# davidfischinger/haf_grasping

Hardware: NVIDIA B200
Metric: grasp_windows_scored_per_sec_all_rolls (higher is better)
Workload: dtype f32 (contraction: fp16 operands, 1 tensor-core product per k-slice, f32 accumulate; f64 guard band)

## Files before the change

haf_grasping_b200/csrc/hafgpu.cu:

```cuda
#include <cuda_runtime.h>

#include <algorithm>
#include <cmath>
#include <cstdarg>
#include <cstdio>
#include <condition_variable>
#include <cstring>
#include <mutex>
#include <unordered_map>
#include <string>
#include <thread>
#include <vector>

#include "../../include/hafgpu.h"
#include "haf_host.hpp"
#include "host/pcd_io.hpp"
#include "kernels.cuh"
#include "pcd_ingest.cuh"
#include "svm_tc.cuh"

using namespace hafk;

static thread_local std::string g_create_error;

// ... 591 lines not shown
        {
            const int forced = (cfg->reserved[0] >> 4) & 3;
            double rel[4] = {0, 0, 0, 0};
            if (!forced || cfg->guard_rel <= 0) calibrate_tensor_passes(model, Dsv, rel);
            int passes = 3;
            if (forced) passes = forced;
            else if (rel[1] <= 5.5e-7) passes = 1;
            else if (rel[2] <= 5.5e-7) passes = 2;
            ctx->tc_passes = passes;
            ctx->tc_operand_err = passes < 3 ? rel[passes] : 0.0;
            if (cfg->guard_rel <= 0) ctx->guard_rel = std::max(4e-6f, (float)(15.0 * (ctx->tc_operand_err + 2.5e-7)));
        }
        if (!make_tensor_map(&ctx->tmSh2, ctx->d_SVh.p, KB, SpadT) || !make_tensor_map(&ctx->tmSl2, ctx->d_SVl.p, KB, SpadT)) {
            haf_destroy(ctx);
            return create_fail(HAF_ERR_CUDA, "cuTensorMapEncodeTiled failed for the support-vector operands");
        }
        std::vector<DimFeat> joined((size_t)32 * D);
        for (int cls = 0; cls < 32; cls++)
        for (int d = 0; d < D; d++) {
            DimFeat j;
            memset(&j, 0, sizeof j);
            const DimDev& dd = dims[d];
            if (dd.feat >= 0) {
                const FeatDev& ff = fd[dd.feat];
                for (int r = 0; r < 3; r++) {
                    if (ff.flags & (1 << r)) {
                        for (int q = 0; q < 4; q++) {
                            const int x = ff.off[4 * r + q] / ld, y = ff.off[4 * r + q] % ld;
                            j.off[4 * r + q] = (x * (ld + cls) + y) * 4;
                        }
                        j.w[r] = ff.w[r];
                    } else {
                        for (int q = 0; q < 4; q++) j.off[4 * r + q] = 0;
                        j.w[r] = 0.0f;
                    }
                }
                j.flags = ff.flags & 0x104;
            } else {
                j.flags = 0x200;
            }
            if (dd.drop) j.flags |= 0x400;
            j.fmin = (float)dd.fmin; j.slope = (float)dd.slope; j.cval = (float)dd.cval;
            joined[(size_t)cls * D + d] = j;
        }
        Round4Tab r4;
        make_round4_table(r4);
        if (ctx->d_round4.ensure(1) != 0) { haf_destroy(ctx); return create_fail(HAF_ERR_NOMEM, "out of device memory uploading the rounding table"); }
        CREATE_TRY(cudaMemcpy(ctx->d_round4.p, &r4, sizeof(Round4Tab), cudaMemcpyHostToDevice));
        if (ctx->d_dimfeat.ensure(joined.size()) != 0) { haf_destroy(ctx); return create_fail(HAF_ERR_NOMEM, "out of device memory uploading the joined feature table"); }
        CREATE_TRY(cudaMemcpy(ctx->d_dimfeat.p, joined.data(), joined.size() * sizeof(DimFeat), cudaMemcpyHostToDevice));
        CREATE_TRY(cudaFuncSetAttribute(haftc::svm_rbf_tc2_kernel, cudaFuncAttributeMaxDynamicSharedMemorySize, haftc::SMEM2_BYTES + haftc::TAB_SMEM_MAX * 4));
        CREATE_TRY(cudaFuncSetAttribute(haftc::svm_rbf_tc3_kernel<2>, cudaFuncAttributeMaxDynamicSharedMemorySize, haftc::TC3_SMEM_LIMIT));
        CREATE_TRY(cudaFuncSetAttribute(haftc::svm_rbf_tc3_kernel<4>, cudaFuncAttributeMaxDynamicSharedMemorySize, haftc::TC3_SMEM_LIMIT));
        CREATE_TRY(cudaFuncSetAttribute(features_tc_kernel, cudaFuncAttributeMaxDynamicSharedMemorySize, (int)ft_smem_layout(G, 2)));
        CREATE_TRY(cudaFuncSetAttribute(features_tc_kernel, cudaFuncAttributePreferredSharedMemoryCarveout, 90));
    }
    for (int i = 0; i < 10; i++) CREATE_TRY(cudaEventCreate(&ctx->ev[i]));
    ctx->ev_ok = true;
#undef CREATE_TRY
    *out = ctx;
    return HAF_OK;
}

extern "C" int haf_create(haf_ctx** out, const haf_config* cfg) {
    if (!out || !cfg) return create_fail(HAF_ERR_ARG, "haf_create: null argument");
    if (cfg->n_devices <= 1) {
        haf_config one = *cfg;
        if (cfg->n_devices == 1 && cfg->devices) one.device = cfg->devices[0];
        one.n_devices = 0; one.devices = nullptr;
        return create_impl(out, &one, false, 0);
    }
    *out = nullptr;
    if (cfg->n_devices > 64) return create_fail(HAF_ERR_ARG, "haf_create: n_devices out of range");
    std::vector<haf_ctx*> members;
    for (int k = 0; k < cfg->n_devices; k++) {
        haf_config one = *cfg;
        one.device = cfg->devices ? cfg->devices[k] : k;
        one.n_devices = 0; one.devices = nullptr;
        for (size_t j = 0; j < members.size(); j++)
            if (members[j]->device == one.device) {
                for (size_t i = 0; i < members.size(); i++) haf_destroy(members[i]);
                return create_fail(HAF_ERR_ARG, "haf_create: devices[] names the same GPU twice");
            }
        haf_ctx* c = nullptr;
        const int rc = create_impl(&c, &one, false, 0);
        if (rc != HAF_OK) {
            for (size_t i = 0; i < members.size(); i++) haf_destroy(members[i]);
            return rc;
        }
        members.push_back(c);
    }
    members[0]->group = members;
    *out = members[0];
    return HAF_OK;
}

static int svm_stage(haf_ctx* ctx, unsigned* cnt, size_t Wcap, size_t ldx, int G, int ubase, cudaStream_t st, cudaEvent_t ev_guard);
extern "C" int haf_svm_create(haf_svm** out, const char* model_path, int device, int svm_mode, int min_dims, float guard_rel) {
    haf_config cfg;
    memset(&cfg, 0, sizeof cfg);
    cfg.model_path = model_path;
    cfg.device = device;
    cfg.svm_mode = svm_mode;
    cfg.guard_rel = guard_rel;
    const int rc = create_impl(out, &cfg, true, min_dims);
    if (rc == HAF_OK) (*out)->svm_only = true;
    return rc;
}
// ... 263 lines not shown

extern "C" int haf_build_transform(const haf_request* req, int roll, int roll_step_deg, float M[16]) {
    if (!req || !M) return HAF_ERR_ARG;
    hafhost::build_transform(*req, roll, roll_step_deg > 0 ? roll_step_deg : 15, M);
    return HAF_OK;
}
extern "C" int haf_build_transform_wcs(const haf_request* req, int roll, int roll_step_deg, float M[16]) {
    if (!req || !M) return HAF_ERR_ARG;
    hafhost::build_transform_wcs(*req, roll, roll_step_deg > 0 ? roll_step_deg : 15, M);
    return HAF_OK;
}
extern "C" int haf_pack_best_records(const haf_best* best, int n, int32_t* records) {
    if (!best || !records || n < 0) return HAF_ERR_ARG;
    for (int i = 0; i < n; i++) {
        int32_t* r = records + (size_t)i * 8;
        r[0] = best[i].topval; r[1] = best[i].row; r[2] = best[i].col; r[3] = best[i].roll; r[4] = best[i].tilt;
        r[5] = best[i].approach_idx; r[6] = best[i].n_windows_scored; r[7] = best[i].rolls_done;
    }
    return HAF_OK;
}
extern "C" uint64_t haf_best_key(int topval, uint32_t unit_order) {
    return ((uint64_t)(uint32_t)(topval + (1 << 30)) << 32) | (uint64_t)(0xFFFFFFFFu - unit_order);
}

namespace {

struct CloudSet {
    const unsigned char* d_xyz;
    size_t stride;
    std::vector<long long> off;
};

long long window_bound(int G, const haf_request& rq) {
    const long long full = (long long)(G - 14) * (G - 14);
    const int ax = (int)rq.area_len_x, ay = (int)rq.area_len_y;
    const long long hr = std::llabs((long long)(ax / 2) - 7), wr = std::llabs((long long)(ay / 2) - 7);
    const long long geo = (2 * hr + 3) * (2 * wr + 3);
    return std::min(full, geo);
}

bool is_pinned_host_ptr(const void* p) {
    cudaPointerAttributes a;
    if (cudaPointerGetAttributes(&a, p) != cudaSuccess) { cudaGetLastError(); return false; }
    return a.type == cudaMemoryTypeHost;
}
bool is_device_ptr(const void* p) {
    cudaPointerAttributes a;
    if (cudaPointerGetAttributes(&a, p) != cudaSuccess) { cudaGetLastError(); return false; }
    return a.type == cudaMemoryTypeDevice || a.type == cudaMemoryTypeManaged;
}

}

static size_t ft_smem_bytes(const haf_ctx* ctx) { return ft_smem_layout(ctx->G, ctx->tc_passes >= 3 ? 2 : 1); }
static size_t exact_smem_bytes(const haf_ctx* ctx) { return (size_t)HAF_EXACT_WB * ctx->Dsv * sizeof(double); }
static int launch_exact(haf_ctx* ctx, ExactArgs a, cudaStream_t st, size_t max_windows) {
    const int slices = (ctx->S + HAF_EXACT_SLICE - 1) / HAF_EXACT_SLICE;
    const size_t passes = a.list ? 1 : (max_windows + a.max_entries - 1) / (size_t)a.max_entries;
    for (size_t p = 0; p < passes; p++) {
        a.entry_begin = (int)(p * (size_t)a.max_entries);
        svm_exact_terms_kernel<<<dim3((unsigned)(ctx->sm_count * 2), (unsigned)slices), 256, exact_smem_bytes(ctx), st>>>(a);
        LAUNCHED(ctx);
        svm_exact_sum_kernel<<<ctx->sm_count * 4, 128, 0, st>>>(a);
        LAUNCHED(ctx);
    }
    return HAF_OK;
}
static ExactArgs make_exact_args(haf_ctx* ctx, const int* list, const unsigned* list_count, unsigned* cnt, int G, int ubase);
static int launch_guard(haf_ctx* ctx, unsigned* cnt, int G, int ubase, cudaStream_t st, size_t Wcap, size_t ldx) {
    if (ctx->tier2_mode == 1) return launch_exact(ctx, make_exact_args(ctx, ctx->d_guardlist.p, cnt + 1, cnt, G, ubase), st, Wcap);
    const size_t cap = std::min<size_t>(ldx, 32768);
    const size_t acc_cap0 = ctx->d_g2accum.cap, tk_cap0 = ctx->d_g2tickets.cap;
    const int ldxg = (int)round_up((size_t)ctx->Dsv, 16);
    ENSURE(ctx, ctx->d_Xg, cap * ldxg); ENSURE(ctx, ctx->d_g2accum, cap * 2); ENSURE(ctx, ctx->d_g2tickets, cap / HAF_G2_WB + 1); ENSURE(ctx, ctx->d_xn64, cap);
    ENSURE(ctx, ctx->d_guardlist2, ldx);
    if (ctx->d_g2accum.cap != acc_cap0) CUDA_TRY(ctx, cudaMemsetAsync(ctx->d_g2accum.p, 0, ctx->d_g2accum.cap * sizeof(double), st));
    if (ctx->d_g2tickets.cap != tk_cap0) CUDA_TRY(ctx, cudaMemsetAsync(ctx->d_g2tickets.p, 0, ctx->d_g2tickets.cap * sizeof(unsigned), st));
    ExactArgs a = make_exact_args(ctx, ctx->d_guardlist.p, cnt + 1, cnt, G, ubase);
    Guard2Args q;
    q.list = ctx->d_guardlist.p; q.list_count = cnt + 1; q.cap = (int)cap; q.Xg = ctx->d_Xg.p; q.svn64 = ctx->d_svn64.p;
    q.ldx = ldxg; q.xn64 = ctx->d_xn64.p;
    q.accum = ctx->d_g2accum.p; q.tickets = ctx->d_g2tickets.p; q.tol2 = ctx->tier2_mode == 2 ? 1e30 : 1e-10;
    q.list2 = ctx->d_guardlist2.p; q.list2_count = cnt + 6;
    const bool audit = ctx->cfg.svm_mode == HAF_SVM_TENSOR_GUARD && ctx->d_dec_tc.p;
    q.dec_tc = audit ? ctx->d_dec_tc.p : nullptr; q.audit_max = cnt + 12; q.guard_flag = audit ? ctx->d_guardflag.p : nullptr;
    const size_t smem = ((size_t)ctx->Dsv * HAF_G2_WB + HAF_G2_WB + 8 * HAF_G2_WB * 2) * sizeof(double);
    const bool few = Wcap < 65536;
    const bool dmma = ctx->tier2_kernel != 2 || smem > 100 * 1024;
    if (few) {
        guard_inputs_flat_kernel<<<32, 256, 0, st>>>(a, q);
        LAUNCHED(ctx);
        if (dmma) { guard_norms_kernel<<<8, 256, 0, st>>>(q); LAUNCHED(ctx); }
    } else {
        guard_inputs_kernel<<<ctx->sm_count * 4, 256, 0, st>>>(a, q);
        LAUNCHED(ctx);
    }
    if (dmma) {
        guard_dmma_kernel<<<(unsigned)ctx->sm_count * 2, 256, HAF_GD_SMEM_BYTES, st>>>(a, q, ctx->Spad / HAF_GD_SB);
    }
    else if (few) guard_fma_kernel<1><<<(unsigned)ctx->sm_count, 256, smem, st>>>(a, q, (ctx->Spad + 255) / 256);
    else guard_fma_kernel<2><<<(unsigned)ctx->sm_count, 256, smem, st>>>(a, q, (ctx->Spad + 511) / 512);
    LAUNCHED(ctx);
    return launch_exact(ctx, make_exact_args(ctx, ctx->d_guardlist2.p, cnt + 6, cnt, G, ubase), st, Wcap);
}
static ExactArgs make_exact_args(haf_ctx* ctx, const int* list, const unsigned* list_count, unsigned* cnt, int G, int ubase) {
    ExactArgs a;
    a.list = list; a.list_count = list_count; a.win_count = cnt + 0; a.integral = ctx->d_integral.p; a.win = ctx->d_win.p;
// ... 422 lines not shown
            if (upg >= 1 && avg_points >= 8 * (long long)GG && (c1 - c0) * 8 >= ctx->sm_count && (ctx->cfg.reserved[1] & 15) != 1) {
                int max_units_per_cloud = 0;
                for (int c = c0; c < c1; c++) max_units_per_cloud = std::max(max_units_per_cloud, std::min(hub[c + 1], ubase + Uc) - std::max(hub[c], ubase));
                const int ug = std::min(upg, std::max(1, max_units_per_cloud));
                int slices = 1;
                {
                    const long long groups = (long long)(c1 - c0) * ((max_units_per_cloud + ug - 1) / ug);
                    const double fixed = std::min(1.0, 4.2 * (double)GG / (double)std::max<long long>(avg_points, 1));
                    double best_cost = 0.0;
                    for (int sl = 1; sl <= 12; sl++) {
                        const double cost = std::ceil((double)(groups * sl) / ctx->sm_count) * (1.0 / sl + fixed);
                        if (sl == 1 || cost < best_cost) { best_cost = cost; slices = sl; }
                    }
                }
                dim3 gridc((unsigned)(c1 - c0), (unsigned)((max_units_per_cloud + ug - 1) / ug), (unsigned)slices);
                if (cs.stride == 12 && (ctx->cfg.reserved[1] & 15) != 2)
                    bin_maxz_cloud_kernel<4><<<gridc, 1024, (size_t)ug * GG * 4, st>>>(cs.d_xyz, cs.stride, d_ptoff + c0, d_cloud_ubegin + c0, d_units,
                                                                                     ctx->d_keys.p - (size_t)ubase * GG, G, r, ug,
                                                                                     reinterpret_cast<unsigned long long*>(cnt + 4), ubase, ubase + Uc);
                else
                    bin_maxz_cloud_kernel<1><<<gridc, 1024, (size_t)ug * GG * 4, st>>>(cs.d_xyz, cs.stride, d_ptoff + c0, d_cloud_ubegin + c0, d_units,
                                                                                     ctx->d_keys.p - (size_t)ubase * GG, G, r, ug,
                                                                                     reinterpret_cast<unsigned long long*>(cnt + 4), ubase, ubase + Uc);
                LAUNCHED(ctx);
            } else {
                const int PPT = 4;
                const long long grid_points = graph_ok ? pts_bucket : max_points;
                dim3 grid((unsigned)((grid_points + 256 * PPT - 1) / (256 * PPT)), (unsigned)(c1 - c0));
                if (grid.x > 0) {
                    bin_maxz_kernel<PPT><<<grid, 256, 0, st>>>(cs.d_xyz, cs.stride, d_ptoff + c0, d_cloud_ubegin + c0, d_units,
                                                               ctx->d_keys.p - (size_t)ubase * GG, G, r, nullptr,
                                                               reinterpret_cast<unsigned long long*>(cnt + 4), ubase, ubase + Uc);
                    LAUNCHED(ctx);
                }
            }
        }
        if (prof) CUDA_TRY(ctx, cudaEventRecord(ctx->ev_pool[ci * 8 + 1], st));
        if (smallG) {
            integral_small_kernel<<<Uc, 128, (size_t)G * ld * sizeof(double), st>>>(ctx->d_keys.p, ctx->d_integral.p, G, units_c);
            LAUNCHED(ctx);
        } else {
            integral_rows_kernel<<<dim3((G + 31) / 32, Uc), 32, 0, st>>>(ctx->d_keys.p, ctx->d_rowscan.p, G, units_c);
            LAUNCHED(ctx);
            integral_cols_kernel<<<dim3((G + 1 + 127) / 128, Uc), 128, 0, st>>>(ctx->d_rowscan.p, ctx->d_integral.p, G, units_c);
            LAUNCHED(ctx);
        }
        if (prof) CUDA_TRY(ctx, cudaEventRecord(ctx->ev_pool[ci * 8 + 2], st));
        mask_windows_kernel<<<dim3((GG + 4095) / 4096, Uc), 256, 0, st>>>(ctx->d_integral.p, units_c, G, ctx->d_mask.p, ctx->d_labelgrid.p,
                                                                         ctx->d_win.p, cnt + 0, (unsigned)Wcap, (int*)(cnt + 2), ubase, d_unit_windows + ubase);
        LAUNCHED(ctx);
        if (prof) CUDA_TRY(ctx, cudaEventRecord(ctx->ev_pool[ci * 8 + 3], st));
        const unsigned wblocks32 = (unsigned)((Wcap + 31) / 32);
        if (tc) {
            const unsigned fblocks = (unsigned)((Wcap + 32 * HAF_FT_WT - 1) / (32 * HAF_FT_WT));
            features_tc_kernel<<<fblocks, 256, ft_smem_bytes(ctx), st>>>(ctx->d_integral.p, ctx->d_win.p, cnt + 0, G, ubase, ctx->d_dimfeat.p, ctx->D,
                                                                      ctx->Krow, (float)ctx->lower, ctx->cfg.emulate_text_roundtrip, ctx->d_round4.p, ctx->d_Xh.p,
                                                                      ctx->tc_passes >= 3 ? ctx->d_Xl.p : nullptr, ctx->d_xn.p, ctx->Dsv, ctx->KB, ctx->d_dec.p, ctx->d_asum.p);
            LAUNCHED(ctx);
        } else if (ctx->cfg.svm_mode != HAF_SVM_FP64_EXACT && !prob) {
            features_kernel<false><<<wblocks32, 256, 0, st>>>(ctx->d_integral.p, ctx->d_win.p, cnt + 0, G, ubase, ctx->d_feats.p, ctx->d_dims.p,
                                                              ctx->D, ctx->Kpad, ctx->lower, ctx->upper, ctx->cfg.emulate_text_roundtrip,
                                                              ctx->d_X.p, ldx, ctx->F, nullptr, nullptr, (int*)(cnt + 3));
            LAUNCHED(ctx);
            xnorm_kernel<<<(unsigned)((Wcap + 255) / 256), 256, 0, st>>>(ctx->d_X.p, ldx, ctx->Kpad, cnt + 0, ctx->d_xn.p);
            LAUNCHED(ctx);
        }
        if (prof) CUDA_TRY(ctx, cudaEventRecord(ctx->ev_pool[ci * 8 + 4], st));
        { int rcs = svm_stage(ctx, cnt, Wcap, ldx, G, ubase, st, prof ? ctx->ev_pool[ci * 8 + 5] : nullptr); if (rcs) return rcs; }
        if (prof) CUDA_TRY(ctx, cudaEventRecord(ctx->ev_pool[ci * 8 + 6], st));
        if (prob) {
            prob_value_kernel<<<(unsigned)((Wcap + 127) / 128), 128, 0, st>>>(ctx->d_dec.p, ctx->d_win.p, cnt + 0, G, ubase, ctx->probA, ctx->probB,
                                                                             ctx->prob_res[0], ctx->prob_res[1], ctx->d_evals.p, (int*)(cnt + 3));
            LAUNCHED(ctx);
            prob_shift_grid_kernel<<<Uc, 1024, 0, st>>>(ctx->d_mask.p, ctx->d_evals.p, G, units_c, ctx->prob_header_val, ctx->d_probgrid.p);
            LAUNCHED(ctx);
            score_prob_kernel<<<dim3((GG + 255) / 256, Uc), 256, 0, st>>>(ctx->d_probgrid.p, G, units_c, ctx->d_evals.p, d_unit_top + ubase);
            LAUNCHED(ctx);
        } else {
            label_scatter_kernel<<<(unsigned)((Wcap + 255) / 256), 256, 0, st>>>(ctx->d_dec.p, ctx->d_win.p, cnt + 0, G, ubase, ctx->gv[0], ctx->gv[1],
                                                                                ctx->d_labelgrid.p);
            LAUNCHED(ctx);
            score_kernel<<<dim3((GG + 255) / 256, Uc), 256, 0, st>>>(ctx->d_labelgrid.p, G, units_c, ctx->d_evals.p, d_unit_top + ubase);
            LAUNCHED(ctx);
        }
        tie_rule_kernel<<<dim3((G + 7) / 8, Uc), 256, 0, st>>>(ctx->d_evals.p, G, units_c, d_unit_top + ubase, d_unit_run + ubase);
        LAUNCHED(ctx);
        if (grasp) {
            grasp_unit_kernel<<<(Uc + 127) / 128, 128, 0, st>>>(ctx->d_keys.p, G, units_c, Uc, d_unit_top + ubase, d_unit_run + ubase, d_pose, d_jpose,
                                                               R, ctx->cfg.roll_step_deg, ctx->d_unit_grasp.p + ubase);
            LAUNCHED(ctx);
        }
        if (prof) CUDA_TRY(ctx, cudaEventRecord(ctx->ev_pool[ci * 8 + 7], st));

        accumulate_counts_kernel<<<1, 1, 0, st>>>(cnt);
        LAUNCHED(ctx);
        if (keep_debug_state) { ctx->last_units = Uc; ctx->last_unit_base = ubase; ctx->last_ldx = ldx; }

        if (out_evals || out_mask || out_heights) {
            for (int j = j0; j < j1; j++) {
                const int na = jobs[j].n_rolls_active - jobs[j].roll_begin;
                if (na <= 0) continue;
                const size_t uo = (size_t)(j * R + jobs[j].roll_begin - ubase) * GG, go = ((size_t)j * R + jobs[j].roll_begin) * GG, nel = (size_t)na * GG;
                if (out_evals) CUDA_TRY(ctx, cudaMemcpyAsync(dst_evals + go, ctx->d_evals.p + uo, nel * 4, cudaMemcpyDefault, st));
                if (out_mask) CUDA_TRY(ctx, cudaMemcpyAsync(dst_mask + go, ctx->d_mask.p + uo, nel, cudaMemcpyDefault, st));
                if (out_heights) CUDA_TRY(ctx, cudaMemcpyAsync(dst_heights + go, ctx->d_keys.p + uo, nel * 4, cudaMemcpyDefault, st));
            }
        }
        if (set) { swap_chunk_ws(ctx, set - 1); ws_scope.set = 0; }
// ... 1009 lines not shown
```

haf_grasping_b200/csrc/kernels.cuh:

```cuda
#pragma once
#include <cuda_fp16.h>
#include <cuda_runtime.h>
#include <stdint.h>

#include "decimal_round.cuh"
#include "haf_host.hpp"

namespace hafk {

struct UnitParams {
    float M[16];
    float sa, ca;
    float cx1, cy1, cx2, cy2, cx3, cy3, cx4, cy4;
    int cloud;
    int job;
    int roll;
    int pad[3];
};
static_assert(sizeof(UnitParams) == 128, "UnitParams layout");

struct __align__(16) FeatDev {
    int off[12];
    float w[3];
    int flags;
// ... 379 lines not shown
    }
    int uns = 0;
    for (int d = warp; d < Kpad; d += 8) {
        double x = 0.0;
        if (d < D && valid) {
            const DimDev dd = dims[d];
            if (dd.feat < 0) {
                x = dd.cval;
            } else {
                const FeatDev f = feats[dd.feat];
                const float raw = feature_value(P, f);
                double v;
                if (emulate_text) {
                    bool u4 = false;
                    v = hafdec::text4(raw, &u4);
                    if (u4) uns = 1;
                } else {
                    v = (double)raw;
                }
                if (dd.drop) x = 0.0;
                else {
                    double val;
                    if (v == dd.fmin) val = lower;
                    else if (v == dd.fmax) val = upper;
                    else val = __dadd_rn(lower, __ddiv_rn(__dmul_rn(__dsub_rn(upper, lower), __dsub_rn(v, dd.fmin)), dd.den));
                    if (val == 0.0) x = 0.0;
                    else if (!emulate_text) x = val;
                    else {
                        bool u6 = false;
                        x = hafdec::text6(val, &u6);
                        if (u6) uns = 1;
                    }
                }
            }
            if (DEBUG && dbg_scaled) dbg_scaled[(size_t)w * D + d] = x;
        }
        if (!DEBUG && valid) X[(size_t)d * ldx + w] = (float)x;
    }
    if (DEBUG && dbg_raw && valid) {
        for (int k = warp; k < F; k += 8) dbg_raw[(size_t)w * F + k] = feature_value(P, feats[k]);
    }
    if (uns) *unsupported_flag = 1;
}

__device__ __forceinline__ double pow10_table(int k) {
    double p = 1.0;
    const int n = k < 0 ? -k : k;
    double b = 10.0;
    int m = n;
    while (m) { if (m & 1) p *= b; b *= b; m >>= 1; }
    return k < 0 ? 1.0 / p : p;
}

#define HAF_FT_ROWS 36

struct __align__(16) DimFeat {
    int off[12];
    float w[3];
    int flags;
    float fmin, slope, cval, padf;
    double pad[2];
};
static_assert(sizeof(DimFeat) == 96, "DimFeat layout");

struct FastTab {
    int off[12];
    float w[3];
    int flags;
    float fmin, slope, cval;
};
__device__ __forceinline__ FastTab load_fast_tab(const DimFeat* __restrict__ table, int d) {
    const uint4* tp = reinterpret_cast<const uint4*>(table + d);
    const uint4 t0 = __ldg(tp), t1 = __ldg(tp + 1), t2 = __ldg(tp + 2), t3 = __ldg(tp + 3), t4 = __ldg(tp + 4);
    FastTab f;
    f.off[0] = (int)t0.x; f.off[1] = (int)t0.y; f.off[2] = (int)t0.z; f.off[3] = (int)t0.w;
    f.off[4] = (int)t1.x; f.off[5] = (int)t1.y; f.off[6] = (int)t1.z; f.off[7] = (int)t1.w;
    f.off[8] = (int)t2.x; f.off[9] = (int)t2.y; f.off[10] = (int)t2.z; f.off[11] = (int)t2.w;
    f.w[0] = __uint_as_float(t3.x); f.w[1] = __uint_as_float(t3.y); f.w[2] = __uint_as_float(t3.z);
    f.flags = (int)t3.w;
    f.fmin = __uint_as_float(t4.x); f.slope = __uint_as_float(t4.y); f.cval = __uint_as_float(t4.z);
    return f;
}
__device__ __forceinline__ FastTab load_fast_tab_smem(uint32_t rec_addr) {
    uint4 t[5];
#pragma unroll
    for (int k = 0; k < 5; k++)
        asm volatile("ld.shared.v4.b32 {%0, %1, %2, %3}, [%4];" : "=r"(t[k].x), "=r"(t[k].y), "=r"(t[k].z), "=r"(t[k].w) : "r"(rec_addr + 16u * k));
    FastTab f;
    f.off[0] = (int)t[0].x; f.off[1] = (int)t[0].y; f.off[2] = (int)t[0].z; f.off[3] = (int)t[0].w;
    f.off[4] = (int)t[1].x; f.off[5] = (int)t[1].y; f.off[6] = (int)t[1].z; f.off[7] = (int)t[1].w;
    f.off[8] = (int)t[2].x; f.off[9] = (int)t[2].y; f.off[10] = (int)t[2].z; f.off[11] = (int)t[2].w;
    f.w[0] = __uint_as_float(t[3].x); f.w[1] = __uint_as_float(t[3].y); f.w[2] = __uint_as_float(t[3].z);
    f.flags = (int)t[3].w;
    f.fmin = __uint_as_float(t[4].x); f.slope = __uint_as_float(t[4].y); f.cval = __uint_as_float(t[4].z);
    return f;
}
struct SmemRows { uint32_t base; };
__device__ __forceinline__ float load_corner(const float* I, int idx0, int off_bytes) {
    return *reinterpret_cast<const float*>(reinterpret_cast<const char*>(I + idx0) + off_bytes);
}
__device__ __forceinline__ float load_corner(SmemRows I, int idx0_bytes, int off_bytes) {
    float v;
    asm volatile("ld.shared.f32 %0, [%1];" : "=f"(v) : "r"(I.base + (uint32_t)(idx0_bytes + off_bytes)));
    return v;
}
struct Round4Tab {
    double pwd[96];
    float pwf[96];
};
static_assert(sizeof(Round4Tab) == 96 * 8 + 96 * 4, "Round4Tab layout");
struct Round4Smem { uint32_t pwd, pwf; };
template <typename PtrT>
__device__ __forceinline__ float fast_tier_value(PtrT I, int idx0, const FastTab& f, float lower, int emulate_text,
                                                 const Round4Smem rt) {
    float c[12];
#pragma unroll
    for (int k = 0; k < 8; k++) c[k] = load_corner(I, idx0, f.off[k]);
    float rr[3];
#pragma unroll
    for (int r = 0; r < 2; r++)
        rr[r] = __fmul_rn(f.w[r], __fadd_rn(__fsub_rn(__fsub_rn(c[4 * r], c[4 * r + 1]), c[4 * r + 2]), c[4 * r + 3]));
    rr[2] = 0.0f;
    if (f.flags & 0x4) {
#pragma unroll
        for (int k = 8; k < 12; k++) c[k] = load_corner(I, idx0, f.off[k]);
        rr[2] = __fmul_rn(f.w[2], __fadd_rn(__fsub_rn(__fsub_rn(c[8], c[9]), c[10]), c[11]));
    }
    float raw;
    if (f.flags & 0x100) {
        const float sa = __fsub_rn(rr[1], rr[0]), sb = __fsub_rn(rr[1], rr[2]);
        raw = (rr[1] > rr[0] && rr[1] > rr[2]) ? ((sb < sa) ? sb : sa) : -1.0f;
    } else {
        raw = __fadd_rn(__fadd_rn(__fadd_rn(0.0f, rr[0]), rr[1]), rr[2]);
    }
    float v = raw;
    if (emulate_text) {
        const float a = fabsf(raw);
        int E = ((max((int)(__float_as_uint(a) >> 23), 1) - 127) * 1233) >> 12;
        float thr;
        asm volatile("ld.shared.f32 %0, [%1];" : "=f"(thr) : "r"(rt.pwf + (uint32_t)((48 + E + 1) << 2)));
        E += (a >= thr) ? 1 : 0;
        double mul; float inv;
        asm volatile("ld.shared.f64 %0, [%1];" : "=d"(mul) : "r"(rt.pwd + (uint32_t)((48 + 3 - E) << 3)));
        asm volatile("ld.shared.f32 %0, [%1];" : "=f"(inv) : "r"(rt.pwf + (uint32_t)((48 + E - 3) << 2)));
        const float r = (float)rint((double)a * mul);
        v = copysignf(r * inv, raw);
    }
    const float x = fmaf(v - f.fmin, f.slope, lower);
    return (f.flags & 0x400) ? 0.0f : ((f.flags & 0x200) ? f.cval : x);
}

__host__ __device__ __forceinline__ size_t kt_off(size_t row, int d, int KB) {
    return (((row >> 7) * (size_t)KB + (size_t)(d >> 6)) << 13) + ((row & 127) << 6) + (size_t)(d & 63);
}
__device__ __forceinline__ void write_aug_columns(__half* __restrict__ X, size_t row, int aug0, int KB, float sq, bool ok) {
    const float a = -0.5f * sq;
    const __half h = __float2half_rn(a);
    const float r1 = a - __half2float(h);
    const __half m = __float2half_rn(r1);
    const __half l = __float2half_rn(r1 - __half2float(m));
    const __half one = __float2half_rn(ok ? 1.0f : 0.0f);
    X[kt_off(row, aug0 + 0, KB)] = h; X[kt_off(row, aug0 + 1, KB)] = m; X[kt_off(row, aug0 + 2, KB)] = l;
    X[kt_off(row, aug0 + 3, KB)] = one; X[kt_off(row, aug0 + 4, KB)] = one; X[kt_off(row, aug0 + 5, KB)] = one;
}

#define HAF_FT_WT 2
#define HAF_FT_KPASS 128
__host__ __device__ constexpr size_t ft_smem_layout(int G, int tiles) {
    return sizeof(Round4Tab) + (size_t)tiles * 32 * HAF_FT_WT * HAF_FT_KPASS * 2 + (size_t)HAF_FT_ROWS * (G + 1 + 31) * 4 + 16 + (size_t)HAF_FT_KPASS * 96;
}
__global__ void __launch_bounds__(256, 4) features_tc_kernel(const float* __restrict__ integral, const int2* __restrict__ win,
                                                             const unsigned* __restrict__ win_count, int G, int unit_base,
                                                             const DimFeat* __restrict__ table, int D, int Krow, float lower,
                                                             int emulate_text, const Round4Tab* __restrict__ rtab,
                                                             __half* __restrict__ Xh, __half* __restrict__ Xl , float* __restrict__ xn,
                                                             int aug0 , int KB ,
                                                             double* __restrict__ dec_acc, float* __restrict__ asum_acc ) {
    constexpr int WT = HAF_FT_WT, NW = 32 * WT;
    extern __shared__ __align__(16) uint32_t s_dyn[];
    static_assert(sizeof(Round4Tab) % 16 == 0, "the tile behind the tables must stay 16-byte aligned");
    uint32_t* const s_words = s_dyn + sizeof(Round4Tab) / 4;
    const int tiles = Xl ? 2 : 1;
    constexpr int TILE_WORDS = NW * HAF_FT_KPASS / 2;
    const unsigned W = *win_count;
    const unsigned w0 = blockIdx.x * NW;
    if (w0 >= W) return;
    const int lane = threadIdx.x & 31;
    const int warp = __shfl_sync(0xffffffffu, (int)(threadIdx.x >> 5), 0);
    const int ld = G + 1;
    float* s_int = reinterpret_cast<float*>(s_words + tiles * TILE_WORDS);
    uint4* s_tab = reinterpret_cast<uint4*>(s_words + ((tiles * TILE_WORDS + HAF_FT_ROWS * (ld + 31) + 3) & ~3));
    __shared__ int s_box[9];
    int unit[WT], row[WT], col[WT];
    bool valid[WT];
#pragma unroll
    for (int t = 0; t < WT; t++) {
        const unsigned w = w0 + t * 32 + lane;
        valid[t] = w < W;
        unit[t] = 0; row[t] = 7; col[t] = 7;
        if (valid[t]) {
            const int2 uc = win[w];
            unit[t] = uc.x;
            row[t] = uc.y / G;
            col[t] = uc.y - row[t] * G;
        }
    }
    if (threadIdx.x < 32) {
        const int uA = __shfl_sync(0xffffffffu, unit[0], 0);
        int uB = uA;
#pragma unroll
        for (int t = 0; t < WT; t++) {
            const unsigned vm = __ballot_sync(0xffffffffu, valid[t]);
            if (vm) uB = __shfl_sync(0xffffffffu, unit[t], 31 - __clz(vm));
        }
        bool two = true;
        int rminA = 0x7fffffff, rmaxA = -1, rminB = 0x7fffffff, rmaxB = -1, cmin = 0x7fffffff, cmax = -1;
#pragma unroll
        for (int t = 0; t < WT; t++) {
            two = two && (!valid[t] || unit[t] == uA || unit[t] == uB);
            if (valid[t]) { cmin = min(cmin, col[t]); cmax = max(cmax, col[t]); }
            if (valid[t] && unit[t] == uA) { rminA = min(rminA, row[t]); rmaxA = max(rmaxA, row[t]); }
            else if (valid[t]) { rminB = min(rminB, row[t]); rmaxB = max(rmaxB, row[t]); }
        }
        two = __all_sync(0xffffffffu, two);
#pragma unroll
        for (int o = 16; o >= 1; o >>= 1) {
            rminA = min(rminA, __shfl_xor_sync(0xffffffffu, rminA, o));
            rmaxA = max(rmaxA, __shfl_xor_sync(0xffffffffu, rmaxA, o));
            rminB = min(rminB, __shfl_xor_sync(0xffffffffu, rminB, o));
            rmaxB = max(rmaxB, __shfl_xor_sync(0xffffffffu, rmaxB, o));
            cmin = min(cmin, __shfl_xor_sync(0xffffffffu, cmin, o));
            cmax = max(cmax, __shfl_xor_sync(0xffffffffu, cmax, o));
        }
        int o = ld;
        bool have = false;
#pragma unroll
        for (int t = 0; t < WT; t++) {
            const int pc = __shfl_up_sync(0xffffffffu, col[t], 1), pr = __shfl_up_sync(0xffffffffu, row[t], 1);
            const int pu = __shfl_up_sync(0xffffffffu, unit[t], 1);
            const bool brk = lane > 0 && valid[t] && pu == unit[t] && row[t] == pr + 1;
            const unsigned m = __ballot_sync(0xffffffffu, brk);
            if (m && !have) { o = __shfl_sync(0xffffffffu, pc + 1 - col[t], __ffs(m) - 1); have = true; }
        }
        if (lane == 0) {
            const int nA = rmaxA - rminA + 15, nB = (uB != uA) ? rmaxB - rminB + 15 : 0;
            const bool ok = two && nA + nB <= HAF_FT_ROWS;
            s_box[0] = uA; s_box[1] = rminA - 7; s_box[2] = ok ? nA : 0;
            s_box[3] = ld + (((o - ld) % 32) + 32) % 32;
            s_box[4] = uB; s_box[5] = rminB - 7; s_box[6] = ok ? nB : 0;
            s_box[7] = cmin - 7; s_box[8] = cmax - cmin + 15;
        }
    }
    for (int t = threadIdx.x; t < (int)(sizeof(Round4Tab) / 8); t += blockDim.x)
        reinterpret_cast<uint2*>(s_dyn)[t] = __ldg(reinterpret_cast<const uint2*>(rtab) + t);
    __syncthreads();
    Round4Smem rt;
    rt.pwd = (uint32_t)__cvta_generic_to_shared(s_dyn);
    asm volatile("" : "+r"(rt.pwd));
    rt.pwf = rt.pwd + (uint32_t)(96 * sizeof(double));
    const int nrows = s_box[2];
    const int sst = nrows > 0 ? s_box[3] : ld;
    table += (size_t)(sst - ld) * D;
    int idx0[WT];
    const float* gI[WT];
#pragma unroll
    for (int t = 0; t < WT; t++) {
        idx0[t] = (row[t] - 7) * ld + (col[t] - 7);
        gI[t] = integral + (size_t)(unit[t] - unit_base) * ld * ld;
    }
    if (nrows > 0) {
        const int nB = s_box[6];
        const float* srcA = integral + (size_t)(s_box[0] - unit_base) * ld * ld + (size_t)s_box[1] * ld;
        const float* srcB = integral + (size_t)(s_box[4] - unit_base) * ld * ld + (size_t)s_box[5] * ld - (size_t)nrows * ld;
        const int c0 = s_box[7], wd = s_box[8];
        for (int t = threadIdx.x; t < (nrows + nB) * wd; t += blockDim.x) {
            const int r = t / wd, c = c0 + (t - r * wd);
            s_int[r * sst + c] = (r < nrows ? srcA : srcB)[r * ld + c];
        }
#pragma unroll
        for (int t = 0; t < WT; t++) {
            const int r0 = (unit[t] == s_box[0]) ? row[t] - 7 - s_box[1] : nrows + row[t] - 7 - s_box[5];
            idx0[t] = valid[t] ? r0 * sst + (col[t] - 7) : 0;
        }
    }
    const uint32_t tab_base = (uint32_t)__cvta_generic_to_shared(s_tab);
    SmemRows srows;
    srows.base = (uint32_t)__cvta_generic_to_shared(s_int);
    float nrm[WT];
#pragma unroll
    for (int t = 0; t < WT; t++) nrm[t] = 0.0f;
    const uint32_t tile_base = rt.pwd + (uint32_t)sizeof(Round4Tab);
    const uint32_t row0 = tile_base + (uint32_t)lane * (HAF_FT_KPASS * 2), row1 = row0 + 32u * (HAF_FT_KPASS * 2);
    const uint32_t sw = (uint32_t)(((lane & 7) << 2) | ((lane >> 3) & 3));
    for (int d0 = 0; d0 < Krow; d0 += HAF_FT_KPASS) {
        const int KP = min(HAF_FT_KPASS, Krow - d0);
        {
            const int nrec = min(KP, D - d0);
            const uint4* src = reinterpret_cast<const uint4*>(table + d0);
            for (int t = threadIdx.x; t < nrec * 6; t += blockDim.x) s_tab[t] = __ldg(src + t);
        }
        __syncthreads();
        for (int dl = warp; dl < KP; dl += 8) {
            const int d = d0 + dl;
            float xf[WT];
#pragma unroll
            for (int t = 0; t < WT; t++) xf[t] = 0.0f;
            if (d < D) {
                const FastTab f = load_fast_tab_smem(tab_base + 96u * dl);
                if (nrows > 0) {
#pragma unroll
                    for (int t = 0; t < WT; t++) xf[t] = fast_tier_value(srows, idx0[t] * 4, f, lower, emulate_text, rt);
                } else {
#pragma unroll
                    for (int t = 0; t < WT; t++) xf[t] = valid[t] ? fast_tier_value(gI[t], idx0[t], f, lower, emulate_text, rt) : 0.0f;
                }
            }
            static_assert(WT == 2, "the packing below converts the two windows of a lane together");
            const __half2 hi2 = __floats2half2_rn(xf[0], xf[1]);
            const float2 hif = __half22float2(hi2);
            const __half2 lo2 = __floats2half2_rn(xf[0] - hif.x, xf[1] - hif.y);
            {
                const float2 lof = __half22float2(lo2);
                const float v0 = hif.x + lof.x, v1 = hif.y + lof.y;
                nrm[0] = fmaf(v0, v0, nrm[0]);
                nrm[1] = fmaf(v1, v1, nrm[1]);
            }
            const uint32_t hu = *reinterpret_cast<const uint32_t*>(&hi2), lu = *reinterpret_cast<const uint32_t*>(&lo2);
            const uint32_t toff = ((((uint32_t)dl >> 1) ^ sw) << 2) | (((uint32_t)dl & 1u) << 1);
            asm volatile("st.shared.b16 [%0], %1;" ::"r"(row0 + toff), "h"((unsigned short)(hu & 0xffffu)) : "memory");
            asm volatile("st.shared.b16 [%0], %1;" ::"r"(row1 + toff), "h"((unsigned short)(hu >> 16)) : "memory");
            if (Xl) {
                asm volatile("st.shared.b16 [%0], %1;" ::"r"(row0 + TILE_WORDS * 4 + toff), "h"((unsigned short)(lu & 0xffffu)) : "memory");
                asm volatile("st.shared.b16 [%0], %1;" ::"r"(row1 + TILE_WORDS * 4 + toff), "h"((unsigned short)(lu >> 16)) : "memory");
            }
        }
        __syncthreads();
        {
            const int c = lane & 15, nch = KP >> 3;
            const size_t coff = ((size_t)((d0 >> 6) + (c >> 3)) << 13) + (size_t)((c & 7) << 3);
#pragma unroll
            for (int k = 0; k < NW / 16; k++) {
                const int wi = 16 * k + 2 * warp + (lane >> 4);
                const unsigned ww = w0 + wi;
                if (ww < W && c < nch) {
                    const uint32_t a = tile_base + (uint32_t)wi * (HAF_FT_KPASS * 2) + (uint32_t)((c ^ (wi & 7)) << 4);
                    const size_t off = ((size_t)(ww >> 7) * (size_t)KB << 13) + ((size_t)(ww & 127) << 6) + coff;
                    const int kx = (wi >> 3) & 3;
#pragma unroll
                    for (int tl = 0; tl < 2; tl++) {
                        if (tl == 1 && !Xl) break;
                        uint4 v;
                        asm volatile("ld.shared.v4.b32 {%0, %1, %2, %3}, [%4];" : "=r"(v.x), "=r"(v.y), "=r"(v.z), "=r"(v.w) : "r"(a + tl * TILE_WORDS * 4));
                        if (kx & 1) { uint32_t t0 = v.x; v.x = v.y; v.y = t0; t0 = v.z; v.z = v.w; v.w = t0; }
                        if (kx & 2) { uint32_t t0 = v.x; v.x = v.z; v.z = t0; t0 = v.y; v.y = v.w; v.w = t0; }
                        *reinterpret_cast<uint4*>((tl ? Xl : Xh) + off) = v;
                    }
                }
            }
        }
    }
    __syncthreads();
    float* s_nrm = reinterpret_cast<float*>(s_words);
#pragma unroll
    for (int t = 0; t < WT; t++) s_nrm[warp * NW + t * 32 + lane] = nrm[t];
    __syncthreads();
    if (threadIdx.x < NW && w0 + threadIdx.x < W) {
        float sq = 0.0f;
#pragma unroll
        for (int k = 0; k < 8; k++) sq += s_nrm[k * NW + threadIdx.x];
        const bool ok = sq < 1.3e5f;
        xn[w0 + threadIdx.x] = ok ? sq : __int_as_float(0x7f800000);
        dec_acc[w0 + threadIdx.x] = 0.0;
        asum_acc[w0 + threadIdx.x] = 0.0f;
        write_aug_columns(Xh, w0 + threadIdx.x, aug0, KB, ok ? sq : 0.0f, ok);
    }
}

__global__ void xnorm_kernel(const float* __restrict__ X, size_t ldx, int Kpad, const unsigned* __restrict__ win_count,
                             float* __restrict__ xn) {
    const unsigned W = *win_count;
    const unsigned w = blockIdx.x * blockDim.x + threadIdx.x;
    if (w >= W) return;
    float s = 0.0f;
    for (int d = 0; d < Kpad; d++) { const float v = X[(size_t)d * ldx + w]; s = fmaf(v, v, s); }
    xn[w] = s;
}
// ... 1080 lines not shown
```

Measured before the change: 345.0 million.

## Template feature kernel on windows per lane and prefetch next dimension's corners

```diff
diff --git a/haf_grasping_b200/csrc/hafgpu.cu b/haf_grasping_b200/csrc/hafgpu.cu
--- a/haf_grasping_b200/csrc/hafgpu.cu
+++ b/haf_grasping_b200/csrc/hafgpu.cu
@@ -667,8 +667,17 @@
         CREATE_TRY(cudaFuncSetAttribute(haftc::svm_rbf_tc2_kernel, cudaFuncAttributeMaxDynamicSharedMemorySize, haftc::SMEM2_BYTES + haftc::TAB_SMEM_MAX * 4));
         CREATE_TRY(cudaFuncSetAttribute(haftc::svm_rbf_tc3_kernel<2>, cudaFuncAttributeMaxDynamicSharedMemorySize, haftc::TC3_SMEM_LIMIT));
         CREATE_TRY(cudaFuncSetAttribute(haftc::svm_rbf_tc3_kernel<4>, cudaFuncAttributeMaxDynamicSharedMemorySize, haftc::TC3_SMEM_LIMIT));
-        CREATE_TRY(cudaFuncSetAttribute(features_tc_kernel, cudaFuncAttributeMaxDynamicSharedMemorySize, (int)ft_smem_layout(G, 2)));
-        CREATE_TRY(cudaFuncSetAttribute(features_tc_kernel, cudaFuncAttributePreferredSharedMemoryCarveout, 90));
+        {
+            size_t need[2] = {0, 0};
+            for (int tiles = 1; tiles <= 2; tiles++) {
+                const int wt = ft_windows_per_lane(G, tiles);
+                need[wt == 4] = std::max(need[wt == 4], ft_smem_layout(G, tiles, wt));
+            }
+            if (need[0]) CREATE_TRY(cudaFuncSetAttribute(features_tc_kernel<2>, cudaFuncAttributeMaxDynamicSharedMemorySize, (int)need[0]));
+            if (need[1]) CREATE_TRY(cudaFuncSetAttribute(features_tc_kernel<4>, cudaFuncAttributeMaxDynamicSharedMemorySize, (int)need[1]));
+        }
+        CREATE_TRY(cudaFuncSetAttribute(features_tc_kernel<2>, cudaFuncAttributePreferredSharedMemoryCarveout, 90));
+        CREATE_TRY(cudaFuncSetAttribute(features_tc_kernel<4>, cudaFuncAttributePreferredSharedMemoryCarveout, 90));
     }
     for (int i = 0; i < 10; i++) CREATE_TRY(cudaEventCreate(&ctx->ev[i]));
     ctx->ev_ok = true;
@@ -1038,7 +1047,6 @@
 
 }
 
-static size_t ft_smem_bytes(const haf_ctx* ctx) { return ft_smem_layout(ctx->G, ctx->tc_passes >= 3 ? 2 : 1); }
 static size_t exact_smem_bytes(const haf_ctx* ctx) { return (size_t)HAF_EXACT_WB * ctx->Dsv * sizeof(double); }
 static int launch_exact(haf_ctx* ctx, ExactArgs a, cudaStream_t st, size_t max_windows) {
     const int slices = (ctx->S + HAF_EXACT_SLICE - 1) / HAF_EXACT_SLICE;
@@ -1567,8 +1575,9 @@
         if (prof) CUDA_TRY(ctx, cudaEventRecord(ctx->ev_pool[ci * 8 + 3], st));
         const unsigned wblocks32 = (unsigned)((Wcap + 31) / 32);
         if (tc) {
-            const unsigned fblocks = (unsigned)((Wcap + 32 * HAF_FT_WT - 1) / (32 * HAF_FT_WT));
-            features_tc_kernel<<<fblocks, 256, ft_smem_bytes(ctx), st>>>(ctx->d_integral.p, ctx->d_win.p, cnt + 0, G, ubase, ctx->d_dimfeat.p, ctx->D,
+            const int ftiles = ctx->tc_passes >= 3 ? 2 : 1, wt = ft_windows_per_lane(G, ftiles);
+            const unsigned fblocks = (unsigned)((Wcap + 32 * wt - 1) / (32 * wt));
+            (wt == 4 ? features_tc_kernel<4> : features_tc_kernel<2>)<<<fblocks, 256, ft_smem_layout(G, ftiles, wt), st>>>(ctx->d_integral.p, ctx->d_win.p, cnt + 0, G, ubase, ctx->d_dimfeat.p, ctx->D,
                                                                       ctx->Krow, (float)ctx->lower, ctx->cfg.emulate_text_roundtrip, ctx->d_round4.p, ctx->d_Xh.p,
                                                                       ctx->tc_passes >= 3 ? ctx->d_Xl.p : nullptr, ctx->d_xn.p, ctx->Dsv, ctx->KB, ctx->d_dec.p, ctx->d_asum.p);
             LAUNCHED(ctx);
diff --git a/haf_grasping_b200/csrc/kernels.cuh b/haf_grasping_b200/csrc/kernels.cuh
--- a/haf_grasping_b200/csrc/kernels.cuh
+++ b/haf_grasping_b200/csrc/kernels.cuh
@@ -455,7 +455,7 @@
     return k < 0 ? 1.0 / p : p;
 }
 
-#define HAF_FT_ROWS 36
+__host__ __device__ constexpr int ft_rows(int wt) { return wt == 4 ? 48 : 36; }
 
 struct __align__(16) DimFeat {
     int off[12];
@@ -513,44 +513,63 @@
 };
 static_assert(sizeof(Round4Tab) == 96 * 8 + 96 * 4, "Round4Tab layout");
 struct Round4Smem { uint32_t pwd, pwf; };
+__device__ __forceinline__ float fast_tier_region(const FastTab& f, int r, const float* c) {
+    return __fmul_rn(f.w[r], __fadd_rn(__fsub_rn(__fsub_rn(c[0], c[1]), c[2]), c[3]));
+}
+__device__ __forceinline__ float fast_tier_combine(const FastTab& f, float r0, float r1, float r2) {
+    if (f.flags & 0x100) {
+        const float sa = __fsub_rn(r1, r0), sb = __fsub_rn(r1, r2);
+        return (r1 > r0 && r1 > r2) ? ((sb < sa) ? sb : sa) : -1.0f;
+    }
+    return __fadd_rn(__fadd_rn(__fadd_rn(0.0f, r0), r1), r2);
+}
+template <int N>
+__device__ __forceinline__ void fast_tier_scale(float (&v)[N], float fmin, float slope, float cval, int flags, float lower,
+                                                int emulate_text, const Round4Smem rt) {
+    if (emulate_text) {
+        int E[N];
+        float thr[N];
+#pragma unroll
+        for (int t = 0; t < N; t++) {
+            E[t] = ((max((int)(__float_as_uint(fabsf(v[t])) >> 23), 1) - 127) * 1233) >> 12;
+            asm volatile("ld.shared.f32 %0, [%1];" : "=f"(thr[t]) : "r"(rt.pwf + (uint32_t)((48 + E[t] + 1) << 2)));
+        }
+        double mul[N];
+        float inv[N];
+#pragma unroll
+        for (int t = 0; t < N; t++) {
+            E[t] += (fabsf(v[t]) >= thr[t]) ? 1 : 0;
+            asm volatile("ld.shared.f64 %0, [%1];" : "=d"(mul[t]) : "r"(rt.pwd + (uint32_t)((48 + 3 - E[t]) << 3)));
+            asm volatile("ld.shared.f32 %0, [%1];" : "=f"(inv[t]) : "r"(rt.pwf + (uint32_t)((48 + E[t] - 3) << 2)));
+        }
+#pragma unroll
+        for (int t = 0; t < N; t++) {
+            const float r = (float)rint((double)fabsf(v[t]) * mul[t]);
+            v[t] = copysignf(r * inv[t], v[t]);
+        }
+    }
+#pragma unroll
+    for (int t = 0; t < N; t++) {
+        const float x = fmaf(v[t] - fmin, slope, lower);
+        v[t] = (flags & 0x400) ? 0.0f : ((flags & 0x200) ? cval : x);
+    }
+}
 template <typename PtrT>
 __device__ __forceinline__ float fast_tier_value(PtrT I, int idx0, const FastTab& f, float lower, int emulate_text,
                                                  const Round4Smem rt) {
     float c[12];
 #pragma unroll
     for (int k = 0; k < 8; k++) c[k] = load_corner(I, idx0, f.off[k]);
-    float rr[3];
-#pragma unroll
-    for (int r = 0; r < 2; r++)
-        rr[r] = __fmul_rn(f.w[r], __fadd_rn(__fsub_rn(__fsub_rn(c[4 * r], c[4 * r + 1]), c[4 * r + 2]), c[4 * r + 3]));
-    rr[2] = 0.0f;
+    const float r0 = fast_tier_region(f, 0, c), r1 = fast_tier_region(f, 1, c + 4);
+    float r2 = 0.0f;
     if (f.flags & 0x4) {
 #pragma unroll
         for (int k = 8; k < 12; k++) c[k] = load_corner(I, idx0, f.off[k]);
-        rr[2] = __fmul_rn(f.w[2], __fadd_rn(__fsub_rn(__fsub_rn(c[8], c[9]), c[10]), c[11]));
-    }
-    float raw;
-    if (f.flags & 0x100) {
-        const float sa = __fsub_rn(rr[1], rr[0]), sb = __fsub_rn(rr[1], rr[2]);
-        raw = (rr[1] > rr[0] && rr[1] > rr[2]) ? ((sb < sa) ? sb : sa) : -1.0f;
-    } else {
-        raw = __fadd_rn(__fadd_rn(__fadd_rn(0.0f, rr[0]), rr[1]), rr[2]);
-    }
-    float v = raw;
-    if (emulate_text) {
-        const float a = fabsf(raw);
-        int E = ((max((int)(__float_as_uint(a) >> 23), 1) - 127) * 1233) >> 12;
-        float thr;
-        asm volatile("ld.shared.f32 %0, [%1];" : "=f"(thr) : "r"(rt.pwf + (uint32_t)((48 + E + 1) << 2)));
-        E += (a >= thr) ? 1 : 0;
-        double mul; float inv;
-        asm volatile("ld.shared.f64 %0, [%1];" : "=d"(mul) : "r"(rt.pwd + (uint32_t)((48 + 3 - E) << 3)));
-        asm volatile("ld.shared.f32 %0, [%1];" : "=f"(inv) : "r"(rt.pwf + (uint32_t)((48 + E - 3) << 2)));
-        const float r = (float)rint((double)a * mul);
-        v = copysignf(r * inv, raw);
-    }
-    const float x = fmaf(v - f.fmin, f.slope, lower);
-    return (f.flags & 0x400) ? 0.0f : ((f.flags & 0x200) ? f.cval : x);
+        r2 = fast_tier_region(f, 2, c + 8);
+    }
+    float v[1] = {fast_tier_combine(f, r0, r1, r2)};
+    fast_tier_scale(v, f.fmin, f.slope, f.cval, f.flags, lower, emulate_text, rt);
+    return v[0];
 }
 
 __host__ __device__ __forceinline__ size_t kt_off(size_t row, int d, int KB) {
@@ -567,19 +586,24 @@
     X[kt_off(row, aug0 + 3, KB)] = one; X[kt_off(row, aug0 + 4, KB)] = one; X[kt_off(row, aug0 + 5, KB)] = one;
 }
 
-#define HAF_FT_WT 2
 #define HAF_FT_KPASS 128
-__host__ __device__ constexpr size_t ft_smem_layout(int G, int tiles) {
-    return sizeof(Round4Tab) + (size_t)tiles * 32 * HAF_FT_WT * HAF_FT_KPASS * 2 + (size_t)HAF_FT_ROWS * (G + 1 + 31) * 4 + 16 + (size_t)HAF_FT_KPASS * 96;
-}
-__global__ void __launch_bounds__(256, 4) features_tc_kernel(const float* __restrict__ integral, const int2* __restrict__ win,
+__host__ __device__ constexpr size_t ft_smem_layout(int G, int tiles, int wt) {
+    return sizeof(Round4Tab) + (size_t)tiles * 32 * wt * HAF_FT_KPASS * 2 + (size_t)ft_rows(wt) * (G + 1 + 31) * 4 + 16 + (size_t)HAF_FT_KPASS * 96;
+}
+__host__ __device__ constexpr int ft_windows_per_lane(int G, int tiles) {
+    return 3 * (ft_smem_layout(G, tiles, 4) + 1024) <= 228 * 1024 ? 4 : 2;
+}
+template <int WT>
+__global__ void __launch_bounds__(256, WT == 4 ? 3 : 4) features_tc_kernel(const float* __restrict__ integral, const int2* __restrict__ win,
                                                              const unsigned* __restrict__ win_count, int G, int unit_base,
                                                              const DimFeat* __restrict__ table, int D, int Krow, float lower,
                                                              int emulate_text, const Round4Tab* __restrict__ rtab,
                                                              __half* __restrict__ Xh, __half* __restrict__ Xl , float* __restrict__ xn,
                                                              int aug0 , int KB ,
                                                              double* __restrict__ dec_acc, float* __restrict__ asum_acc ) {
-    constexpr int WT = HAF_FT_WT, NW = 32 * WT;
+    static_assert(WT == 2 || WT == 4, "the fp16 packing below converts pairs of windows");
+    constexpr int NW = 32 * WT, ROWS = ft_rows(WT);
+    constexpr int NPRE = WT / 2;
     extern __shared__ __align__(16) uint32_t s_dyn[];
     static_assert(sizeof(Round4Tab) % 16 == 0, "the tile behind the tables must stay 16-byte aligned");
     uint32_t* const s_words = s_dyn + sizeof(Round4Tab) / 4;
@@ -592,7 +616,7 @@
     const int warp = __shfl_sync(0xffffffffu, (int)(threadIdx.x >> 5), 0);
     const int ld = G + 1;
     float* s_int = reinterpret_cast<float*>(s_words + tiles * TILE_WORDS);
-    uint4* s_tab = reinterpret_cast<uint4*>(s_words + ((tiles * TILE_WORDS + HAF_FT_ROWS * (ld + 31) + 3) & ~3));
+    uint4* s_tab = reinterpret_cast<uint4*>(s_words + ((tiles * TILE_WORDS + ROWS * (ld + 31) + 3) & ~3));
     __shared__ int s_box[9];
     int unit[WT], row[WT], col[WT];
     bool valid[WT];
@@ -647,7 +671,7 @@
         }
         if (lane == 0) {
             const int nA = rmaxA - rminA + 15, nB = (uB != uA) ? rmaxB - rminB + 15 : 0;
-            const bool ok = two && nA + nB <= HAF_FT_ROWS;
+            const bool ok = two && nA + nB <= ROWS;
             s_box[0] = uA; s_box[1] = rminA - 7; s_box[2] = ok ? nA : 0;
             s_box[3] = ld + (((o - ld) % 32) + 32) % 32;
             s_box[4] = uB; s_box[5] = rminB - 7; s_box[6] = ok ? nB : 0;
@@ -665,12 +689,8 @@
     const int sst = nrows > 0 ? s_box[3] : ld;
     table += (size_t)(sst - ld) * D;
     int idx0[WT];
-    const float* gI[WT];
-#pragma unroll
-    for (int t = 0; t < WT; t++) {
-        idx0[t] = (row[t] - 7) * ld + (col[t] - 7);
-        gI[t] = integral + (size_t)(unit[t] - unit_base) * ld * ld;
-    }
+#pragma unroll
+    for (int t = 0; t < WT; t++) idx0[t] = (row[t] - 7) * ld + (col[t] - 7);
     if (nrows > 0) {
         const int nB = s_box[6];
         const float* srcA = integral + (size_t)(s_box[0] - unit_base) * ld * ld + (size_t)s_box[1] * ld;
@@ -683,7 +703,7 @@
 #pragma unroll
         for (int t = 0; t < WT; t++) {
             const int r0 = (unit[t] == s_box[0]) ? row[t] - 7 - s_box[1] : nrows + row[t] - 7 - s_box[5];
-            idx0[t] = valid[t] ? r0 * sst + (col[t] - 7) : 0;
+            idx0[t] = valid[t] ? (r0 * sst + (col[t] - 7)) * 4 : 0;
         }
     }
     const uint32_t tab_base = (uint32_t)__cvta_generic_to_shared(s_tab);
@@ -693,48 +713,97 @@
 #pragma unroll
     for (int t = 0; t < WT; t++) nrm[t] = 0.0f;
     const uint32_t tile_base = rt.pwd + (uint32_t)sizeof(Round4Tab);
-    const uint32_t row0 = tile_base + (uint32_t)lane * (HAF_FT_KPASS * 2), row1 = row0 + 32u * (HAF_FT_KPASS * 2);
+    const uint32_t row0 = tile_base + (uint32_t)lane * (HAF_FT_KPASS * 2);
     const uint32_t sw = (uint32_t)(((lane & 7) << 2) | ((lane >> 3) & 3));
     for (int d0 = 0; d0 < Krow; d0 += HAF_FT_KPASS) {
         const int KP = min(HAF_FT_KPASS, Krow - d0);
+        const int nrec = min(KP, D - d0);
         {
-            const int nrec = min(KP, D - d0);
             const uint4* src = reinterpret_cast<const uint4*>(table + d0);
             for (int t = threadIdx.x; t < nrec * 6; t += blockDim.x) s_tab[t] = __ldg(src + t);
         }
         __syncthreads();
+        FastTab f;
+        float c[WT][8];
+        if (nrows > 0 && warp < nrec) {
+            f = load_fast_tab_smem(tab_base + 96u * warp);
+#pragma unroll
+            for (int t = 0; t < NPRE; t++)
+#pragma unroll
+                for (int k = 0; k < 8; k++) c[t][k] = load_corner(srows, idx0[t], f.off[k]);
+        }
         for (int dl = warp; dl < KP; dl += 8) {
-            const int d = d0 + dl;
             float xf[WT];
 #pragma unroll
             for (int t = 0; t < WT; t++) xf[t] = 0.0f;
-            if (d < D) {
-                const FastTab f = load_fast_tab_smem(tab_base + 96u * dl);
+            if (dl < nrec) {
                 if (nrows > 0) {
 #pragma unroll
-                    for (int t = 0; t < WT; t++) xf[t] = fast_tier_value(srows, idx0[t] * 4, f, lower, emulate_text, rt);
+                    for (int t = NPRE; t < WT; t++)
+#pragma unroll
+                        for (int k = 0; k < 8; k++) c[t][k] = load_corner(srows, idx0[t], f.off[k]);
+                    float r0[WT], r1[WT], r2[WT];
+#pragma unroll
+                    for (int t = 0; t < WT; t++) {
+                        r0[t] = fast_tier_region(f, 0, c[t]);
+                        r1[t] = fast_tier_region(f, 1, c[t] + 4);
+                        r2[t] = 0.0f;
+                    }
+                    if (f.flags & 0x4) {
+                        float c3[WT][4];
+#pragma unroll
+                        for (int t = 0; t < WT; t++)
+#pragma unroll
+                            for (int k = 0; k < 4; k++) c3[t][k] = load_corner(srows, idx0[t], f.off[8 + k]);
+#pragma unroll
+                        for (int t = 0; t < WT; t++) r2[t] = fast_tier_region(f, 2, c3[t]);
+                    }
+                    if (f.flags & 0x100) {
+#pragma unroll
+                        for (int t = 0; t < WT; t++) xf[t] = fast_tier_combine(f, r0[t], r1[t], r2[t]);
+                    } else {
+#pragma unroll
+                        for (int t = 0; t < WT; t++) xf[t] = fast_tier_combine(f, r0[t], r1[t], r2[t]);
+                    }
+                    const float fmin = f.fmin, slope = f.slope, cval = f.cval;
+                    const int flags = f.flags;
+                    if (dl + 8 < nrec) {
+                        f = load_fast_tab_smem(tab_base + 96u * (dl + 8));
+#pragma unroll
+                        for (int t = 0; t < NPRE; t++)
+#pragma unroll
+                            for (int k = 0; k < 8; k++) c[t][k] = load_corner(srows, idx0[t], f.off[k]);
+                    }
+                    fast_tier_scale(xf, fmin, slope, cval, flags, lower, emulate_text, rt);
                 } else {
-#pragma unroll
-                    for (int t = 0; t < WT; t++) xf[t] = valid[t] ? fast_tier_value(gI[t], idx0[t], f, lower, emulate_text, rt) : 0.0f;
+                    const FastTab fg = load_fast_tab_smem(tab_base + 96u * dl);
+#pragma unroll
+                    for (int t = 0; t < WT; t++) {
+                        const unsigned w = w0 + t * 32 + lane;
+                        if (w < W) xf[t] = fast_tier_value(integral + (size_t)(unit[t] - unit_base) * ld * ld, idx0[t], fg, lower, emulate_text, rt);
+                    }
                 }
             }
-            static_assert(WT == 2, "the packing below converts the two windows of a lane together");
-            const __half2 hi2 = __floats2half2_rn(xf[0], xf[1]);
-            const float2 hif = __half22float2(hi2);
-            const __half2 lo2 = __floats2half2_rn(xf[0] - hif.x, xf[1] - hif.y);
-            {
-                const float2 lof = __half22float2(lo2);
-                const float v0 = hif.x + lof.x, v1 = hif.y + lof.y;
-                nrm[0] = fmaf(v0, v0, nrm[0]);
-                nrm[1] = fmaf(v1, v1, nrm[1]);
-            }
-            const uint32_t hu = *reinterpret_cast<const uint32_t*>(&hi2), lu = *reinterpret_cast<const uint32_t*>(&lo2);
             const uint32_t toff = ((((uint32_t)dl >> 1) ^ sw) << 2) | (((uint32_t)dl & 1u) << 1);
-            asm volatile("st.shared.b16 [%0], %1;" ::"r"(row0 + toff), "h"((unsigned short)(hu & 0xffffu)) : "memory");
-            asm volatile("st.shared.b16 [%0], %1;" ::"r"(row1 + toff), "h"((unsigned short)(hu >> 16)) : "memory");
-            if (Xl) {
-                asm volatile("st.shared.b16 [%0], %1;" ::"r"(row0 + TILE_WORDS * 4 + toff), "h"((unsigned short)(lu & 0xffffu)) : "memory");
-                asm volatile("st.shared.b16 [%0], %1;" ::"r"(row1 + TILE_WORDS * 4 + toff), "h"((unsigned short)(lu >> 16)) : "memory");
+#pragma unroll
+            for (int p = 0; p < WT; p += 2) {
+                const __half2 hi2 = __floats2half2_rn(xf[p], xf[p + 1]);
+                const float2 hif = __half22float2(hi2);
+                const __half2 lo2 = __floats2half2_rn(xf[p] - hif.x, xf[p + 1] - hif.y);
+                {
+                    const float2 lof = __half22float2(lo2);
+                    const float v0 = hif.x + lof.x, v1 = hif.y + lof.y;
+                    nrm[p] = fmaf(v0, v0, nrm[p]);
+                    nrm[p + 1] = fmaf(v1, v1, nrm[p + 1]);
+                }
+                const uint32_t hu = *reinterpret_cast<const uint32_t*>(&hi2), lu = *reinterpret_cast<const uint32_t*>(&lo2);
+                const uint32_t ra = row0 + (uint32_t)p * (32u * HAF_FT_KPASS * 2) + toff, rb = ra + 32u * (HAF_FT_KPASS * 2);
+                asm volatile("st.shared.b16 [%0], %1;" ::"r"(ra), "h"((unsigned short)(hu & 0xffffu)) : "memory");
+                asm volatile("st.shared.b16 [%0], %1;" ::"r"(rb), "h"((unsigned short)(hu >> 16)) : "memory");
+                if (Xl) {
+                    asm volatile("st.shared.b16 [%0], %1;" ::"r"(ra + TILE_WORDS * 4), "h"((unsigned short)(lu & 0xffffu)) : "memory");
+                    asm volatile("st.shared.b16 [%0], %1;" ::"r"(rb + TILE_WORDS * 4), "h"((unsigned short)(lu >> 16)) : "memory");
+                }
             }
         }
         __syncthreads();
```

New measurement: 355.7 million, median of 6. 1.03x the previous value.
